# kvas7andy/unreal

Measured on AMD Instinct MI355X. Metric: env-steps/sec (whole node), UNREAL maze 84x84, higher is better.
Workload: dtype f32 (fp16x2-split MFMA operands, fp32 accumulate)

## Files before the change

include/unreal_hip.h:

```cpp
#ifndef UNREAL_HIP_H
#define UNREAL_HIP_H
#include <stdint.h>
#ifdef __cplusplus
extern "C" {
#endif

#define UNREAL_FRAME_BYTES 21168
#define UNREAL_PC_CELLS 400
#define UNREAL_GEMM_RELU 1
#define UNREAL_GEMM_ACCUM 2
#define UNREAL_GEMM_ATOMIC 4
#define UNREAL_GEMM_RELU_MASK 8
#define UNREAL_GEMM_RELU_BITS 16

int unreal_maze_step(int B, int H1, const int* actions, const int* active, int* pos, int* last_action,
                     float* last_reward, int* count, uint8_t* frames, float* r_reward, int* r_action,
                     int* r_terminal, int* r_last_action, float* r_last_reward, float* r_pc,
                     float* out_reward, int* out_terminal, float* episode_reward, float* score_out,
                     int* score_valid, int reset_on_terminal, int track_score, void* stream);
int unreal_maze_rollout_step(int B, int H1, const int* actions, int* pos, int* last_action, float* last_reward, int* count,
                             uint8_t* frames, float* r_reward, int* r_action, int* r_terminal, int* r_last_action,
                             float* r_last_reward, float* r_pc, float* out_reward, int* out_terminal,
                             float* episode_reward, float* score_out, int* score_valid, int* active,
                             int* active_log_t, int* n_steps, int* terminal_end, int* next_idx ,
// ... 88 lines not shown
int unreal_encoder_hw_fwd(int N, int H, int W, const uint8_t* frames, long frame_stride, const int* frame_idx,
                          float frame_scale, const float* W1, const float* b1, const float* W2, const float* b2,
                          float* c1_out, float* f2_out, float* f2_absmax, void* stream);
int unreal_encoder_hw_bwd(int N, int H, int W, const uint8_t* frames, long frame_stride, const int* frame_idx,
                          float frame_scale, const float* W2, const float* c1_saved, const float* d2, float* work,
                          long work_floats, float* dW1, float* db1, float* dW2, float* db2, void* stream);
int unreal_encoder_hw_work_floats(int N, int H, int W, long* out, void* stream);

int unreal_gemm_f32(int transA, int transB, int M, int N, int K, const float* A, int lda, const float* B,
                    int ldb, float* C, int ldc, const float* bias, const float* mask, int ldm, int flags,
                    int splitk, void* stream);
int unreal_absmax_f32(int rows, int cols, const float* x, int ld, float* slot, void* stream);
int unreal_gemm_f32_split_nt(int M, int N, int K, const float* A, int lda, const float* a_absmax, const uint16_t* W2,
                             int ldw, long plane_stride, const float* w_absmax, float* C, int ldc, float* c_absmax,
                             const float* bias,
                             const void* mask ,
                             int ldm, int flags, int splitk, void* stream);
int unreal_gemm_f32_split_nt_slabs(int M, int N, int K, const float* A, int lda, const float* a_absmax, const uint16_t* W3,
                                   int ldw, long plane_stride, const float* w_absmax, float* C, int ldc, float* c_absmax,
                                   const float* bias, int flags, int splitk, float* partials, long partial_floats,
                                   void* stream);
int unreal_gemm_f32_split_tn(int M, int N, int K, const float* A, int lda, const float* a_absmax, const float* B, int ldb,
                             const float* b_absmax, float* C, int ldc, float* colsum, int splitk, void* stream);
int unreal_shadow_refresh_multi(const void* abs_descs, int n_abs, int abs_blocks, const void* split_descs, int n_split,
                                int split_blocks, void* stream);
int unreal_split_f16x2(int rows, int cols, const float* src, int ld_src, int transpose, int row_perm, uint16_t* dst,
                       int ld_dst, long plane_stride, const float* w_absmax, void* stream);
int unreal_lstm_step_fwd(int rows, const float* x, int ldx, int Kx, const float* x_absmax, const float* h_prev, int ld_hprev,
                         const uint16_t* W2, int ldw, long plane_stride, const float* w_absmax, float* gates,
                         const float* bias, const float* c_prev, float* c_out, float* h_out, int ld_h, void* stream);
int unreal_lstm_bptt_step(int rows, const float* d_gates, const float* a_absmax, const uint16_t* Wh2, int ldw,
                          long plane_stride, const float* w_absmax, const float* dh_above, float* dc_io,
                          const float* gates_act, const float* c_prev, const float* c_new, float* dpre,
                          float* dpre_absmax0, float* dpre_absmax1, void* stream);
int unreal_lstm_gates_fwd(int rows, const float* pre, const float* bias, const float* c_prev, float* gates_act,
                          float* c_out, float* h_out, int ld_h, void* stream);
int unreal_lstm_gates_bwd(int rows, const float* dh_above, const float* dh_rec, float* dc_io, const float* gates_act,
                          const float* c_prev, const float* c_new, float* dpre, float* dpre_absmax0 ,
                          float* dpre_absmax1 , void* stream);

int unreal_linear_small_fwd(int rows, int K, int NOUT, const float* X, int ldx, const float* W, const float* b,
                            float* out, int ldo, void* stream);
int unreal_linear_small_bwd(int rows, int K, int NOUT, const float* X, int ldx, const float* dO, int ldo,
                            const float* W, float* dX, int lddx, int accumulate_dx, float* dW, int dw_stride_k,
                            int dw_stride_n, float* db, void* stream);
int unreal_softmax_sample(int rows, int A, float* logits_pi, int ld, const double* u, int* action, void* stream);
// ... 38 lines not shown
```

unreal_amd/csrc/gemm_split.hip:

```cpp
#include "common.h"

namespace {

constexpr int BK = 32;
constexpr int NPL = 2;
typedef _Float16 f16x8 __attribute__((ext_vector_type(8)));
typedef _Float16 f16x2 __attribute__((ext_vector_type(2)));
constexpr int ROW_B = 80;
constexpr int FLAG_RELU = 1, FLAG_ACCUM = 2, FLAG_ATOMIC = 4, FLAG_RELU_MASK = 8, FLAG_RELU_BITS = 16;

typedef float f32x2 __attribute__((ext_vector_type(2)));
typedef unsigned int u32x2 __attribute__((ext_vector_type(2)));
typedef unsigned int u32x4 __attribute__((ext_vector_type(4)));

__device__ __forceinline__ int row_deal(int j) { return (j & ~7) | ((j & 1) << 2) | ((j >> 1) & 3); }

struct SplitArgs {
  int M, N, K;
  const float* A; int lda;
  const unsigned short* W; int ldw; long plane;
  float* C; int ldc;
  const float* bias;
  const float* mask; int ldm;
  int flags;
// ... 463 lines not shown
  }
  if (p.c_absmax0) {
    float* wmx0 = reinterpret_cast<float*>(smem_all + C_BYTES);
    omax = wave_max(omax);
    if ((threadIdx.x & 63) == 0) wmx0[threadIdx.x >> 6] = omax;
    __syncthreads();
    if (threadIdx.x < 64) {
      float m = wmx0[0];
#pragma unroll
      for (int g = 1; g < 4 * KW; ++g) m = fmaxf(m, wmx0[g]);
      absmax_commit(p.c_absmax0, m);
    }
  }
}

struct SplitTnArgs {
  int M, N, K;
  const float* A; int lda;
  const float* B; int ldb;
  float* C; int ldc;
  float* colsum;
  int ntx, nty, splitk, ktiles_per_split;
  const float* a_absmax; const float* b_absmax;
};

__device__ __forceinline__ int tn_m4() {
  const int t = threadIdx.x;
  return ((t >> 1) & 1) | (((t >> 4) & 1) << 1) | (((t >> 2) & 3) << 2) | (((t >> 5) & 1) << 4);
}
__device__ __forceinline__ int tn_k4() {
  const int t = threadIdx.x;
  return (t & 1) | ((t >> 6) << 1);
}

__device__ __forceinline__ void tn_piece_load(const float* __restrict__ P, int ld, int K, int c0, int k0, f32x4 (&reg)[4]) {
  const int m4 = tn_m4(), k4 = tn_k4();
  const int col = min(c0 + 4 * m4, ld - 4);
#pragma unroll
  for (int kk = 0; kk < 4; ++kk) {
    const int k = min(k0 + 4 * k4 + kk, K - 1);
    reg[kk] = *reinterpret_cast<const f32x4*>(P + (size_t)k * ld + col);
  }
}

template <int ROWS, bool RAGGED>
__device__ __forceinline__ void tn_piece_store(unsigned char* S, const f32x4 (&reg)[4], int klim, float scale) {
// ... 5 lines not shown
  for (int j = 0; j < 4; ++j) {
    const int r = 4 * m4 + j;
    u32x2 pl[NPL];
    split4_terms(ok[0] ? reg[0][j] * scale : 0.f, ok[1] ? reg[1][j] * scale : 0.f, ok[2] ? reg[2][j] * scale : 0.f,
                 ok[3] ? reg[3][j] * scale : 0.f, pl);
    const int off = (((k4 >> 1) ^ ((r >> 4) & 3)) * 2 + (k4 & 1)) * 8;
#pragma unroll
    for (int t = 0; t < NPL; ++t)
      *reinterpret_cast<u32x2*>(S + (t * ROWS + r) * ROW_B + off) = pl[t];
  }
}

template <bool RAGGED>
__device__ __forceinline__ void tn_colsum_acc(const f32x4 (&reg)[4], int klim, float w, float (&cs)[4]) {
  const int k4 = tn_k4();
#pragma unroll
  for (int kk = 0; kk < 4; ++kk) {
    const float wk = (!RAGGED || 4 * k4 + kk < klim) ? w : 0.f;
#pragma unroll
    for (int j = 0; j < 4; ++j) cs[j] = fmaf(wk, reg[kk][j], cs[j]);
  }
}

template <bool RAGGED>
__global__ __launch_bounds__(256, 2) void gemm_split_tn_kernel(SplitTnArgs p) {
  constexpr int BM = 128, BN = 128, TM = 2, TN = 2;
  constexpr int A_BYTES = NPL * BM * ROW_B, B_BYTES = NPL * BN * ROW_B;
  constexpr int OP_BYTES = A_BYTES + B_BYTES;
  __shared__ __attribute__((aligned(16))) unsigned char smem[OP_BYTES > 8 * BN * 4 ? OP_BYTES : 8 * BN * 4];
  const float SA = pow2_scale(*p.a_absmax), SB = pow2_scale(*p.b_absmax);
  const float INV_A = pow2_inv(SA), INV_B = pow2_inv(SB);
  unsigned char* As = smem;
  unsigned char* Bs = smem + A_BYTES;

  const int L = blockIdx.x, xcd = L & 7, s = L >> 3;
  const int tiles = p.ntx * p.nty;
  const int slab = (s / tiles) * 8 + xcd, tile = s % tiles;
  if (slab >= p.splitk) return;
  const int bx = tile % p.ntx, by = tile / p.ntx;
  const int m0 = by * BM, n0 = bx * BN;
  const int nk_total = (p.K + BK - 1) / BK;
  const int kt0 = slab * p.ktiles_per_split, kt1 = min(nk_total, kt0 + p.ktiles_per_split);
  if (kt0 >= kt1) return;
  const int nkt = kt1 - kt0;
  const int lane = threadIdx.x & 63, wave = threadIdx.x >> 6;
  const int wm = wave >> 1, wn = wave & 1;
  const int li = lane & 31, kh = lane >> 5;

  f32x16 acc[TM][TN];
#pragma unroll
  for (int i = 0; i < TM; ++i)
#pragma unroll
    for (int j = 0; j < TN; ++j)
#pragma unroll
      for (int r = 0; r < 16; ++r) acc[i][j][r] = 0.f;

  constexpr int TN_FLUSH = 8;
  f32x16 tot[TM][TN];
#pragma unroll
  for (int i = 0; i < TM; ++i)
#pragma unroll
    for (int j = 0; j < TN; ++j)
#pragma unroll
      for (int r = 0; r < 16; ++r) tot[i][j][r] = 0.f;
  f32x4 ra[4], rb[4];
  const float csw = (p.colsum != nullptr && by == 0) ? 1.f : 0.f;
  float cs[4] = {0.f, 0.f, 0.f, 0.f};
  tn_piece_load(p.A, p.lda, p.K, m0, kt0 * BK, ra);
  tn_piece_load(p.B, p.ldb, p.K, n0, kt0 * BK, rb);
  tn_piece_store<BM, RAGGED>(As, ra, p.K - kt0 * BK, SA);
  tn_piece_store<BN, RAGGED>(Bs, rb, p.K - kt0 * BK, SB);
  tn_colsum_acc<RAGGED>(rb, p.K - kt0 * BK, csw, cs);
  {
    const int k1 = (kt0 + min(1, nkt - 1)) * BK;
    tn_piece_load(p.A, p.lda, p.K, m0, k1, ra);
    tn_piece_load(p.B, p.ldb, p.K, n0, k1, rb);
  }
  __syncthreads();

  for (int it = 0; it < nkt; ++it) {
    f16x8 af[TM][NPL], bf[TN][NPL];
    read_frags<BM, BN, true>(As, Bs, wm, wn, li, kh, 0, af, bf);
    mma_frags<TM, TN>(af, bf, acc);
    read_frags<BM, BN, true>(As, Bs, wm, wn, li, kh, 1, af, bf);
    __syncthreads();
    const int kcur = (kt0 + min(it + 1, nkt - 1)) * BK, knext = (kt0 + min(it + 2, nkt - 1)) * BK;
    tn_piece_store<BM, RAGGED>(As, ra, p.K - kcur, SA);
    tn_piece_load(p.A, p.lda, p.K, m0, knext, ra);
    tn_piece_store<BN, RAGGED>(Bs, rb, p.K - kcur, SB);
    tn_colsum_acc<RAGGED>(rb, p.K - kcur, (it + 1 < nkt) ? csw : 0.f, cs);
    tn_piece_load(p.B, p.ldb, p.K, n0, knext, rb);
    mma_frags<TM, TN>(af, bf, acc);
    if ((it + 1) % TN_FLUSH == 0) {
#pragma unroll
      for (int i = 0; i < TM; ++i)
#pragma unroll
        for (int j = 0; j < TN; ++j)
#pragma unroll
          for (int r = 0; r < 16; ++r) { tot[i][j][r] += acc[i][j][r]; acc[i][j][r] = 0.f; }
    }
    __syncthreads();
  }
#pragma unroll
  for (int i = 0; i < TM; ++i)
#pragma unroll
    for (int j = 0; j < TN; ++j)
#pragma unroll
      for (int r = 0; r < 16; ++r) acc[i][j][r] += tot[i][j][r];

  if (csw != 0.f) {
    float* red = reinterpret_cast<float*>(smem);
    const int m4 = tn_m4(), k4 = tn_k4();
#pragma unroll
    for (int j = 0; j < 4; ++j) red[k4 * BN + 4 * m4 + j] = cs[j];
    __syncthreads();
    if (threadIdx.x < BN && n0 + threadIdx.x < p.N) {
      float v = 0.f;
#pragma unroll
      for (int k = 0; k < 8; ++k) v += red[k * BN + threadIdx.x];
      atomicAdd(p.colsum + n0 + threadIdx.x, v);
    }
  }
#pragma unroll
  for (int i = 0; i < TM; ++i)
#pragma unroll
// ... 9 lines not shown
}

__global__ __launch_bounds__(256) void split_planes_f16x2_kernel(int rows, int cols, const float* __restrict__ src, int ld_src,
                                                                 int transpose, unsigned short* __restrict__ dst, int ld_dst,
                                                                 long plane, int row_perm, const float* __restrict__ w_absmax) {
  __shared__ float t[32][33];
  const float sw = pow2_scale(*w_absmax);
  const int c0 = blockIdx.x * 32, r0 = blockIdx.y * 32;
  const int tx = threadIdx.x & 31, ty = threadIdx.x >> 5;
  for (int y = ty; y < 32; y += 8)
    if (r0 + y < rows && c0 + tx < cols) t[y][tx] = src[(size_t)(r0 + y) * ld_src + c0 + tx];
  __syncthreads();
  for (int y = ty; y < 32; y += 8) {
    int orow = transpose ? c0 + y : r0 + y;
    const int ocol = transpose ? r0 + tx : c0 + tx;
    if (row_perm == 1) orow = ((orow & 255) >> 4) * 64 + (orow >> 8) * 16 + (orow & 15);
    const bool ok = transpose ? (c0 + y < cols && r0 + tx < rows) : (r0 + y < rows && c0 + tx < cols);
    if (!ok) continue;
    const float x = (transpose ? t[tx][y] : t[y][tx]) * sw;
    const _Float16 h = (_Float16)x;
    const _Float16 l = (_Float16)(x - (float)h);
    dst[(size_t)orow * ld_dst + ocol] = __builtin_bit_cast(unsigned short, h);
    dst[plane + (size_t)orow * ld_dst + ocol] = __builtin_bit_cast(unsigned short, l);
  }
}

__global__ __launch_bounds__(256) void absmax_kernel(int rows, int cols, const float* __restrict__ x, int ld, float* slot) {
  float m = 0.f;
  if (ld == cols && (cols & 3) == 0 && ((((uintptr_t)x) & 15) == 0)) {
    const long n4 = (long)rows * cols / 4;
    const f32x4* x4 = reinterpret_cast<const f32x4*>(x);
    for (long i = (long)blockIdx.x * 256 + threadIdx.x; i < n4; i += (long)gridDim.x * 256) {
      const f32x4 v = x4[i];
      m = fmaxf(fmaxf(m, fmaxf(fabsf(v[0]), fabsf(v[1]))), fmaxf(fabsf(v[2]), fabsf(v[3])));
    }
  } else {
    const int wave = (blockIdx.x * 256 + threadIdx.x) >> 6, nw = (gridDim.x * 256) >> 6, lane = threadIdx.x & 63;
    for (int r = wave; r < rows; r += nw)
      for (int c = lane; c < cols; c += 64) m = fmaxf(m, fabsf(x[(size_t)r * ld + c]));
  }
  __shared__ float wm[4];
  m = wave_max(m);
  if ((threadIdx.x & 63) == 0) wm[threadIdx.x >> 6] = m;
  __syncthreads();
  if (threadIdx.x < 64) absmax_commit(slot, fmaxf(fmaxf(wm[0], wm[1]), fmaxf(wm[2], wm[3])));
}
// ... 292 lines not shown
  a.bias = nullptr; a.mask = nullptr; a.ldm = 0; a.flags = 0; a.vecA = 1;
  a.c_prev = c_prev; a.c_out = nullptr; a.h_out = nullptr; a.ld_h = 0;
  a.A2 = nullptr; a.lda2 = 0; a.K1 = 1024; a.K1pad = 0;
  a.dh_above = dh_above; a.dc_io = dc_io; a.gates_act = gates_act; a.c_new = c_new; a.dpre = dpre;
  a.a_absmax = a_absmax; a.a_floor = 0.f; a.w_absmax = w_absmax; a.c_absmax0 = dpre_absmax0; a.c_absmax1 = dpre_absmax1;
  a.splitk = 1; a.ktiles_per_split = 1024 / BK; a.slab_stride = 0;
  a.nbx = 4; a.nby = (rows + 63) / 64;
  const int grid = a.nbx * ((a.nby + 7) / 8 * 8);
  const long tiles = (long)a.nbx * a.nby;
  const int kw = tiles <= 256 ? 4 : tiles <= 512 ? 2 : 1;
  if (kw == 4) {
    UNREAL_LAUNCHED("bptt kw4");
    hipLaunchKernelGGL((gemm_split_nt_kernel<64, 64, true, 2, 4>), dim3(grid), dim3(1024), 0, (hipStream_t)stream, a);
  } else if (kw == 2) {
    UNREAL_LAUNCHED("bptt kw2");
    hipLaunchKernelGGL((gemm_split_nt_kernel<64, 64, true, 2, 2>), dim3(grid), dim3(512), 0, (hipStream_t)stream, a);
  } else {
    UNREAL_LAUNCHED("bptt kw1");
    hipLaunchKernelGGL((gemm_split_nt_kernel<64, 64, true, 2, 1>), dim3(grid), dim3(256), 0, (hipStream_t)stream, a);
  }
  return unreal_launch_status();
}

int unreal_gemm_f32_split_tn(int M, int N, int K, const float* A, int lda, const float* a_absmax, const float* B, int ldb,
                             const float* b_absmax, float* C, int ldc, float* colsum, int splitk, void* stream) {
  if (M <= 0 || N <= 0 || K <= 0 || !A || !B || !C || lda < M || ldb < N || ldc < N) return UNREAL_EINVAL;
  if ((lda & 3) || (ldb & 3) || lda < 4 || ldb < 4 || (((uintptr_t)A) & 15) || (((uintptr_t)B) & 15)) return UNREAL_EINVAL;
  SplitTnArgs a;
  a.M = M; a.N = N; a.K = K; a.A = A; a.lda = lda; a.B = B; a.ldb = ldb; a.C = C; a.ldc = ldc; a.colsum = colsum;
  a.a_absmax = a_absmax; a.b_absmax = b_absmax;
  if (!a.a_absmax || !a.b_absmax) return UNREAL_EINVAL;
  a.ntx = (N + 127) / 128; a.nty = (M + 127) / 128;
  const int nk = (K + BK - 1) / BK;
  if (splitk < 1) splitk = 1;
  if (splitk > nk) splitk = nk;
  a.ktiles_per_split = (nk + splitk - 1) / splitk;
  a.splitk = (nk + a.ktiles_per_split - 1) / a.ktiles_per_split;
  const long grid = (long)a.ntx * a.nty * ((a.splitk + 7) / 8 * 8);
  if (grid > 0x7fffffffL) return UNREAL_EINVAL;
  if (K % BK == 0) {
    UNREAL_LAUNCHED("split_tn even");
    hipLaunchKernelGGL(gemm_split_tn_kernel<false>, dim3((unsigned)grid), dim3(256), 0, (hipStream_t)stream, a);
  } else {
    UNREAL_LAUNCHED("split_tn ragged");
    hipLaunchKernelGGL(gemm_split_tn_kernel<true>, dim3((unsigned)grid), dim3(256), 0, (hipStream_t)stream, a);
  }
  return unreal_launch_status();
}

}
```

unreal_amd/model/model.py:

```python
import math
from collections import OrderedDict

import numpy as np
import torch

from .. import ops

ALIGN = 64
XLD = 264


def xcat_ld(action_size, objective_size=0):
    return max(XLD, (256 + action_size + 1 + objective_size + 7) // 8 * 8)


def _small_chunks(n):
    out = []
    while n > 0:
        w = n if n in (1, 3, 4, 5, 6, 7) else (1 if n == 2 else (7 if n >= 10 else n - 3 if n - 3 in (3, 4, 5, 6) else 4))
        out.append(w)
        n -= w
    return out


# ... 59 lines not shown
        self.frame_idx = torch.zeros(rows, dtype=torch.int32, device=device)
        self.c1 = f(rows * c1_dim) if save_c1 else None
        self.f2 = f(rows * f2_dim)
        self.f2_bits = torch.zeros(rows * ops.RELU_WORDS, dtype=torch.int16, device=device) \
            if save_c1 and f2_dim == ops.F2_DIM and c1_dim == ops.C1_DIM else None
        self.xcat = torch.zeros(rows * xld, dtype=torch.float32, device=device)
        if lstm:
            self.gates = f(rows * 1024)
            self.c = f(rows * 256)
            self.h = f(rows * 256)
            self.c0 = torch.zeros(B * 256, dtype=torch.float32, device=device)
            self.h0 = torch.zeros(B * 256, dtype=torch.float32, device=device)


class GradWS(object):

    def __init__(self, rows, B, device, lstm=True, pc=True, A=4, pc_rows=None, f2_dim=ops.F2_DIM):
        f = lambda n: torch.empty(n, dtype=torch.float32, device=device)
        pc_rows = rows if pc_rows is None else pc_rows
        self.f2_dim = f2_dim
        self.d_feat = f(rows * 256)
        self.d_fc = f(rows * 256)
        self.d_f2 = f(rows * f2_dim)
        if lstm:
            self.d_gates = f(rows * 1024)
            self.dh_rec = f(B * 256)
            self.dc = f(B * 256)
        self.rows, self.lstm, self.device = rows, lstm, device
        self.hp = self.d_hp = self.d_dec = self.pc_R = None
        if pc:
            self.ensure_pc(pc_rows, A, own_d_hp=pc_rows != rows)

    def ensure_pc(self, pc_rows, A, own_d_hp=False):
        if self.hp is not None and self.hp.numel() >= pc_rows * ops.F2_DIM:
            return
        f = lambda n: torch.empty(n, dtype=torch.float32, device=self.device)
        self.hp = f(pc_rows * ops.F2_DIM)
        self.d_hp = f(pc_rows * ops.F2_DIM) if own_d_hp else None
        self.d_dec = None
        self.pc_R = f(pc_rows * ops.PC_CELLS)

    def ensure_d_dec(self, pc_rows, A):
        n = pc_rows * ops.PC_CELLS * (1 + A)
        if self.d_dec is None or self.d_dec.numel() < n:
            self.d_dec = torch.empty(n, dtype=torch.float32, device=self.device)
        return self.d_dec

    def ensure_rows(self, rows, B, device):
        if rows <= self.rows:
            return
        f = lambda n: torch.empty(n, dtype=torch.float32, device=device)
        self.rows = rows
        self.d_feat, self.d_fc, self.d_f2 = f(rows * 256), f(rows * 256), f(rows * self.f2_dim)
        if self.lstm:
            self.d_gates = f(rows * 1024)


def _splitk(M, N, K):
    tiles = ((M + 127) // 128) * ((N + 127) // 128)
    nk = (K + 31) // 32
    if nk < 64:
        return max(1, min(nk // 4 if nk >= 8 else 1, (1024 + tiles - 1) // tiles))
    return max(8, min(8 * int(round(128.0 / tiles)), nk // 4 // 8 * 8))


class UnrealModel(object):

    def __init__(self, action_size, objective_size, thread_index, use_lstm, use_pixel_change,
                 use_value_replay, use_reward_prediction, pixel_change_lambda, entropy_beta, device,
                 segnet_param_dict=None, image_shape=(84, 84), is_training=True, n_classes=0,
                 segnet_lambda=1.0, dropout=0.0, for_display=False, frame_scale=None, seed=0):
        if objective_size < 0:
            raise ValueError("objective_size must be >= 0")
        if segnet_param_dict is not None and segnet_param_dict.get("segnet_mode", 0) not in (0, None):
            raise NotImplementedError("only the vanilla encoder (segnet_mode == 0) is on the hot path")
        self.image_shape = (int(image_shape[0]), int(image_shape[1]))
# ... 329 lines not shown
                              splitk=_splitk(256, 1024, rows), colsum=g["lstm_bias"],
                              a_max=ws.s_x, b_max=s_all)
            c0 = 256
            for w in _small_chunks(K_x - 256):
                ops.linear_small_bwd(rows, 1024, w, gws.d_gates, 1024, ws.xcat[c0:], self.xld, None, None, 0, False,
                                     dW[c0 * 1024:], None, dw_stride_k=1, dw_stride_n=1024)
                c0 += w
            if T > 1:
                r1 = (T - 1) * B
                ops.gemm_split_tn(256, 1024, r1, ws.h, 256, gws.d_gates[B * 1024:], 1024, dW[K_x * 1024:], 1024,
                              splitk=_splitk(256, 1024, r1), a_max=self._one, b_max=s_all)
            if h0_nonzero:
                ops.gemm_split_tn(256, 1024, B, ws.h0, 256, gws.d_gates, 1024, dW[K_x * 1024:], 1024,
                              splitk=_splitk(256, 1024, B), a_max=self._one, b_max=s_all)
            s_dfc = self.new_slot()
            ops.gemm_split_nt(rows, 256, 1024, gws.d_gates, 1024, sh["lstm_fc_dgrad"], gws.d_fc, 256, mask=ws.xcat,
                              ldm=self.xld, flags=ops.GEMM_RELU_MASK, a_max=s_all, c_max=s_dfc)
            d_fc = gws.d_fc
        else:
            ops.relu_mask(rows, 256, d_feat, 256, ws.xcat, self.xld)
            d_fc = d_feat
            s_dfc = ops.absmax(rows, 256, d_fc, 256, self.new_slot())
        F = self.F
        ops.gemm_split_tn(F, 256, rows, ws.f2, F, d_fc, 256, g["W_base_fc1"], 256,
                              splitk=_splitk(F, 256, rows), colsum=g["b_base_fc1"], a_max=ws.s_f2, b_max=s_dfc)
        s_df2 = self.new_slot()
        if ws.f2_bits is not None and self.relu_bits:
            ops.gemm_split_nt(rows, F, 256, d_fc, 256, sh["fc1_dgrad"], gws.d_f2, F, mask=ws.f2_bits,
                              ldm=ops.RELU_WORDS, flags=ops.GEMM_RELU_BITS, a_max=s_dfc, c_max=s_df2)
        else:
            ops.gemm_split_nt(rows, F, 256, d_fc, 256, sh["fc1_dgrad"], gws.d_f2, F, mask=ws.f2, ldm=F,
                              flags=ops.GEMM_RELU_MASK, a_max=s_dfc, c_max=s_df2)
        self.encoder_backward(ring, ws.frame_idx[:rows], ws.c1, gws.d_f2, c1_max=ws.s_c1, d2_max=s_df2)

    def heads_forward(self, rows, feat, ld, pi_out, v_out):
        p, A = self.p, self._action_size
        ops.linear_small_fwd(rows, 256, A, feat, ld, p["W_base_fc_p"], p["b_base_fc_p"], pi_out, A)
        ops.linear_small_fwd(rows, 256, 1, feat, ld, p["W_base_fc_v"], p["b_base_fc_v"], v_out, 1)

    def policy_step(self, rows, feat, ld, u, pi_out, v_out, actions_out):
        p = self.p
        ops.policy_step(rows, self._action_size, feat, ld, p["W_base_fc_p"], p["b_base_fc_p"], p["W_base_fc_v"],
                        p["b_base_fc_v"], u, pi_out, v_out, actions_out)

    def value_forward(self, rows, feat, ld, v_out):
        p = self.p
        ops.linear_small_fwd(rows, 256, 1, feat, ld, p["W_base_fc_v"], p["b_base_fc_v"], v_out, 1)

# ... 104 lines not shown
```

unreal_amd/ops.py:

```python
import torch

from ._lib import lib, ptr, stream

FRAME_BYTES = 21168
PC_CELLS = 400
F2_DIM = 2592
C1_DIM = 6400
GEMM_RELU, GEMM_ACCUM, GEMM_ATOMIC, GEMM_RELU_MASK, GEMM_RELU_BITS = 1, 2, 4, 8, 16
RELU_WORDS = 162

FRAME_SHAPE = (84, 84)
FRAME_HW_MIN, FRAME_HW_MAX = 20, 480


def frame_dims(H, W):
    H, W = int(H), int(W)
    if not (FRAME_HW_MIN <= H <= FRAME_HW_MAX and FRAME_HW_MIN <= W <= FRAME_HW_MAX):
        raise ValueError("frame size %dx%d: supported are %d <= H, W <= %d" % (H, W, FRAME_HW_MIN, FRAME_HW_MAX))
    h1, w1 = (H - 8) // 4 + 1, (W - 8) // 4 + 1
    h2, w2 = (h1 - 4) // 2 + 1, (w1 - 4) // 2 + 1
    return h1, w1, h2, w2, 32 * h2 * w2


def frame_stride(H, W):
# ... 615 lines not shown


def gemm_split_nt_slabs(M, N, K, A, lda, W, C, ldc, partials, splitk, bias=None, flags=0, a_max=None, c_max=None):
    if W.N != N or W.K != K:
        raise ValueError("split weights are [%d,%d], GEMM wants [%d,%d]" % (W.N, W.K, N, K))
    _chk(A, "f32", (M - 1) * lda + K, "A"); _chk(C, "f32", (M - 1) * ldc + N, "C")
    _chk(bias, "f32", N, "bias", optional=True); _chk(partials, "f32", splitk * M * ((N + 3) // 4 * 4), "partials")
    _chk(a_max, "f32", 1, "a_max", optional=True); _chk(c_max, "f32", 1, "c_max", optional=True)
    a_max = _absmax_of(A, M, K, lda, a_max)
    _call("unreal_gemm_f32_split_nt_slabs", M, N, K, ptr(A), lda, ptr(a_max), ptr(W.planes), W.ldw, W.plane, ptr(W.wmax), ptr(C),
          ldc, ptr(c_max), ptr(bias), flags, splitk, ptr(partials), partials.numel())


def gemm_split_tn(M, N, K, A, lda, B, ldb, C, ldc, splitk=1, colsum=None, a_max=None, b_max=None):
    _chk(A, "f32", (K - 1) * lda + M, "A"); _chk(B, "f32", (K - 1) * ldb + N, "B"); _chk(C, "f32", (M - 1) * ldc + N, "C")
    _chk(colsum, "f32", N, "colsum", optional=True)
    _chk(a_max, "f32", 1, "a_max", optional=True); _chk(b_max, "f32", 1, "b_max", optional=True)
    a_max = _absmax_of(A, K, M, lda, a_max)
    b_max = _absmax_of(B, K, N, ldb, b_max)
    _call("unreal_gemm_f32_split_tn", M, N, K, ptr(A), lda, ptr(a_max), ptr(B), ldb, ptr(b_max), ptr(C), ldc, ptr(colsum),
          splitk)


def lstm_step_fwd(rows, h_prev, Wh, gates, bias, c_prev, c_out, h_out, ld_hprev=256, ld_h=256, x=None, ldx=0, Kx=0,
                  x_max=None):
    kxpad = (Kx + 31) // 32 * 32 if x is not None else 0
    if Wh.N != 1024 or Wh.K != kxpad + 256 or Wh.row_perm != 1:
        raise ValueError("lstm_step_fwd needs the gate-interleaved [1024,%d] shadow of the LSTM kernel" % (kxpad + 256))
    _chk(h_prev, "f32", (rows - 1) * ld_hprev + 256, "h_prev"); _chk(gates, "f32", rows * 1024, "gates")
    _chk(bias, "f32", 1024, "bias"); _chk(c_prev, "f32", rows * 256, "c_prev"); _chk(c_out, "f32", rows * 256, "c_out")
    _chk(h_out, "f32", (rows - 1) * ld_h + 256, "h_out")
    _chk(x, "f32", (rows - 1) * ldx + Kx if x is not None else None, "x", optional=True)
    _chk(x_max, "f32", 1, "x_max", optional=True)
    if x is not None:
        x_max = _absmax_of(x, rows, Kx, ldx, x_max)
    _call("unreal_lstm_step_fwd", rows, ptr(x), ldx, Kx, ptr(x_max), ptr(h_prev), ld_hprev, ptr(Wh.planes), Wh.ldw, Wh.plane,
          ptr(Wh.wmax), ptr(gates), ptr(bias), ptr(c_prev), ptr(c_out), ptr(h_out), ld_h)


def lstm_gates_fwd(rows, pre, bias, c_prev, gates_act, c_out, h_out, ld_h=256):
    _chk(pre, "f32", rows * 1024); _chk(bias, "f32", 1024); _chk(c_prev, "f32", rows * 256)
    _chk(gates_act, "f32", rows * 1024, optional=True); _chk(c_out, "f32", rows * 256)
    _chk(h_out, "f32", (rows - 1) * ld_h + 256)
    _call("unreal_lstm_gates_fwd", rows, ptr(pre), ptr(bias), ptr(c_prev), ptr(gates_act), ptr(c_out), ptr(h_out),
          ld_h)

# ... 149 lines not shown
```

unreal_amd/train/trainer.py:

```python
import time

import torch

from .. import ops
from ..environment.environment import Environment
from ..environment.maze_environment import BatchedMazeEnvironment
from ..model.model import UnrealModel, PathWS, GradWS
from .experience import Experience

PERFORMANCE_LOG_INTERVAL = 2000


def log_uniform(lo, hi, rate):
    import math
    return math.exp(math.log(lo) * (1 - rate) + math.log(hi) * rate)


class PhiloxDraws(object):

    def __init__(self, seed, rank=0, batch=None, world_size=1):
        self.seed = int(seed)
        self.counter = 1
        self.batch = None if batch is None else int(batch)
        self.stride = None if batch is None else int(batch) * int(world_size)
# ... 469 lines not shown
                          g["W_pc_deconv_v"], g["b_pc_deconv_v"], g["W_pc_deconv_a"], g["b_pc_deconv_a"], dhp_max=s_dhp,
                          hp_max=s_hp, ddec_max=s_dd)
        return s_dhp

    def _train_pc(self):
        B, Ta, A, net = self.Bg, self.local_t_max, self.action_size, self.local_network
        p, g, gws = net.p, net.g, self.gws
        rows = Ta * B
        ws = self.aux_ws
        gws.ensure_pc(rows, A)
        feat, ld = self._sample_sequence()
        s_bhp = net.new_slot()
        net.pc_head_forward(B, feat, ld, self.boot_hp, ws=self.boot_ws, hp_max=s_bhp)
        ops.pc_deconv_fwd(B, A, self.boot_hp, p["W_pc_deconv_v"], p["b_pc_deconv_v"], p["W_pc_deconv_a"],
                          p["b_pc_deconv_a"], qmax=self.boot_qmax, hp_max=s_bhp)
        ops.pc_returns(self.ring, Ta + 1, self.seq_idx, self.seq_len, self.boot_qmax, self.gamma_pc, gws.pc_R)
        feat, ld = self._aux_forward()
        s_hp = net.new_slot()
        net.pc_head_forward(rows, feat, ld, gws.hp, ws=self.aux_ws, hp_max=s_hp)
        ops.gather_i32(self.ring.r_action, self.aux_ws.frame_idx[:rows], self.seq_act)
        d_hp = gws.d_f2
        s_dhp = self._pc_deconv_loss_backward(gws, rows, self.seq_mask, d_hp, s_hp)
        from ..model.model import _splitk
        ops.gemm_split_tn(256, 2592, rows, feat, ld, d_hp, 2592, g["W_pc_fc1"], 2592,
                              splitk=_splitk(256, 2592, rows), colsum=g["b_pc_fc1"],
                              a_max=net._one if self.use_lstm else self.aux_ws.s_x, b_max=s_dhp)
        ops.gemm_split_nt(rows, 256, 2592, d_hp, 2592, net.shadow["pc_fc1_dgrad"], gws.d_feat, 256, a_max=s_dhp)
        net.trunk_backward(self.ring, self.aux_ws, gws, Ta, B, gws.d_feat)

    def _train_vr(self):
        B, Ta, net = self.Bg, self.local_t_max, self.local_network
        p, g, gws = net.p, net.g, self.gws
        rows = Ta * B
        ws = self.aux_ws
        feat, ld = self._sample_sequence()
        net.value_forward(B, feat, ld, self.aux_boot_v)
        ops.vr_returns(self.ring, Ta + 1, self.seq_idx, self.seq_len, self.aux_boot_v, self.gamma, self.aux_R)
        feat, ld = self._aux_forward()
        net.value_forward(rows, feat, ld, self.aux_v)
        ops.vr_loss_grad(rows, self.aux_v, self.aux_R, self.seq_mask, self.grad_scale, self.dv, self.losses[4:5])
        ops.linear_small_bwd(rows, 256, 1, feat, ld, self.dv, 1, p["W_base_fc_v"], gws.d_feat, 256, False,
                             g["W_base_fc_v"], g["b_base_fc_v"])
        net.trunk_backward(self.ring, self.aux_ws, gws, Ta, B, gws.d_feat)

    batch_aux_default = True

    def _train_aux_batched(self):
        B, Ta, A, net = self.Bg, self.local_t_max, self.action_size, self.local_network
        p, g, gws, sh = net.p, net.g, self.gws2, net.shadow
# ... 3 lines not shown
            ops.replay_sample_seq(self.ring, L, self.seq_start2[s], self.seq_idx2[s], self.seq_len2[s])
            ops.seq_last_idx(B, self.seq_idx2[s], self.seq_len2[s], self.last2[s * B:(s + 1) * B])
            ops.seq_mask(B, Ta, self.seq_len2[s], self.seq_mask2[s])
        bw = self.boot2_ws
        ops.gather_i32(self.last2, self.map_boot, bw.frame_idx[:2 * B])
        feat, ld = net.trunk_forward(self.ring, bw, 1, 2 * B, lar_from_ring=True, save_c1=False)
        s_bhp = net.new_slot()
        net.pc_head_forward(B, feat, 2 * ld, self.boot_hp, ws=self.boot2_ws, hp_max=s_bhp)
        ops.pc_deconv_fwd(B, A, self.boot_hp, p["W_pc_deconv_v"], p["b_pc_deconv_v"], p["W_pc_deconv_a"],
                          p["b_pc_deconv_a"], qmax=self.boot_qmax, hp_max=s_bhp)
        ops.pc_returns(self.ring, L, self.seq_idx2[0], self.seq_len2[0], self.boot_qmax, self.gamma_pc, gws.pc_R)
        net.value_forward(B, feat[ld:], 2 * ld, self.aux_boot_v)
        ops.vr_returns(self.ring, L, self.seq_idx2[1], self.seq_len2[1], self.aux_boot_v, self.gamma, self.aux_R)
        ws = self.aux2_ws
        ops.gather_i32(self.seq_idx_cat, self.map_seq, ws.frame_idx[:2 * rows])
        feat, ld = net.trunk_forward(self.ring, ws, Ta, 2 * B, lar_from_ring=True, save_c1=True)
        d_feat = gws.d_feat
        s_hp = net.new_slot()
        net.pc_head_forward(rows, feat, 2 * ld, gws.hp, ws=self.aux2_ws, hp_max=s_hp)
        ops.gather_i32(self.ring.r_action, self.seq_idx2[0][:rows], self.seq_act)
        d_hp = gws.d_hp
        s_dhp = self._pc_deconv_loss_backward(gws, rows, self.seq_mask2[0], d_hp, s_hp)
        from ..model.model import _splitk
        ops.gemm_split_tn(256, 2592, rows, feat, 2 * ld, d_hp, 2592, g["W_pc_fc1"], 2592,
                          splitk=_splitk(256, 2592, rows), colsum=g["b_pc_fc1"],
                          a_max=net._one if self.use_lstm else self.aux2_ws.s_x, b_max=s_dhp)
        ops.gemm_split_nt(rows, 256, 2592, d_hp, 2592, sh["pc_fc1_dgrad"], d_feat, 2 * 256, a_max=s_dhp)
        net.value_forward(rows, feat[ld:], 2 * ld, self.aux_v)
        ops.vr_loss_grad(rows, self.aux_v, self.aux_R, self.seq_mask2[1], self.grad_scale, self.aux_dv, self.losses[4:5])
        ops.linear_small_bwd(rows, 256, 1, feat[ld:], 2 * ld, self.aux_dv, 1, p["W_base_fc_v"], d_feat[256:], 2 * 256, False,
                             g["W_base_fc_v"], g["b_base_fc_v"])
        net.trunk_backward(self.ring, ws, gws, Ta, 2 * B, d_feat)

    def _train_rp(self):
        B, net, ws = self.Bg, self.local_network, self.rp_ws
        p, g, gws = net.p, net.g, self.gws
        self.draws.randint(2, self.rp_coin)
        self.draws.uniform(self.rp_u)
        ops.replay_sample_rp(self.ring, self.rp_coin, self.rp_u, ws.frame_idx[:3 * B], self.rp_class, self.rp_mode)
        s_c1 = net.new_slot()
        F = net.F
        net.encoder_forward(self.ring, ws.frame_idx[:3 * B], ws.f2, ws.c1, c1_max=s_c1, ws=ws)
        ops.linear_small_fwd(B, 3 * F, 3, ws.f2, 3 * F, p["W_rp_fc1"], p["b_rp_fc1"], self.rp_logits, 3)
        ops.rp_loss_grad(B, self.rp_logits, self.rp_class, self.grad_scale, None, self.rp_dlogits,
                         self.losses[5:6])
        ops.linear_small_bwd(B, 3 * F, 3, ws.f2, 3 * F, self.rp_dlogits, 3, p["W_rp_fc1"], gws.d_f2, 3 * F, False,
                             g["W_rp_fc1"], g["b_rp_fc1"])
        ops.relu_mask(3 * B, F, gws.d_f2, F, ws.f2, F)
        net.encoder_backward(self.ring, ws.frame_idx[:3 * B], ws.c1, gws.d_f2,
# ... 92 lines not shown
```

Baseline: 3.762 million.

## Pre-split narrow activation operand into fp16x2 planes for weight-gradient TN GEMMs

Adds a kernel that transposes a narrow (256-wide) fp32 activation or gradient matrix once into K-contiguous fp16 hi/lo planes, optionally folding in the bias column sum. The TN weight-gradient GEMM gains template variants that load the pre-split planes directly into shared memory instead of re-splitting fp32 tiles in every block. This targets the redundant split and transposed fp32 loads repeated across the wide grid dimension. The cost is an extra launch and a plane buffer write and read.

```diff
diff --git a/include/unreal_hip.h b/include/unreal_hip.h
--- a/include/unreal_hip.h
+++ b/include/unreal_hip.h
@@ -134,6 +134,11 @@
                                    void* stream);
 int unreal_gemm_f32_split_tn(int M, int N, int K, const float* A, int lda, const float* a_absmax, const float* B, int ldb,
                              const float* b_absmax, float* C, int ldc, float* colsum, int splitk, void* stream);
+int unreal_split_act_f16x2(int K, int N, const float* src, int ld_src, const float* absmax, uint16_t* dst, int ld_dst,
+                           long plane_stride, float* colsum, void* stream);
+int unreal_gemm_f32_split_tn_planes(int M, int N, int K, const float* A, int lda, const uint16_t* Ap, int ldap, long a_plane,
+                                    const float* a_absmax, const float* B, int ldb, const uint16_t* Bp, int ldbp, long b_plane,
+                                    const float* b_absmax, float* C, int ldc, float* colsum, int splitk, void* stream);
 int unreal_shadow_refresh_multi(const void* abs_descs, int n_abs, int abs_blocks, const void* split_descs, int n_split,
                                 int split_blocks, void* stream);
 int unreal_split_f16x2(int rows, int cols, const float* src, int ld_src, int transpose, int row_perm, uint16_t* dst,
diff --git a/unreal_amd/csrc/gemm_split.hip b/unreal_amd/csrc/gemm_split.hip
--- a/unreal_amd/csrc/gemm_split.hip
+++ b/unreal_amd/csrc/gemm_split.hip
@@ -509,6 +509,8 @@
   float* colsum;
   int ntx, nty, splitk, ktiles_per_split;
   const float* a_absmax; const float* b_absmax;
+  const unsigned short* Ap; int ldap; long a_plane;
+  const unsigned short* Bp; int ldbp; long b_plane;
 };
 
 __device__ __forceinline__ int tn_m4() {
@@ -560,7 +562,22 @@
   }
 }
 
-template <bool RAGGED>
+__device__ __forceinline__ void tn_planes_load(const unsigned short* __restrict__ P, int ld, long plane, int rows_total, int r0,
+                                               int k0, u32x4 (&reg)[4]) {
+#pragma unroll
+  for (int q = 0; q < 4; ++q) reg[q] = w_piece_load<128>(P, ld, plane, rows_total, r0, k0, q, threadIdx.x);
+}
+
+__device__ __forceinline__ void tn_planes_store(unsigned char* S, const u32x4 (&reg)[4]) {
+#pragma unroll
+  for (int q = 0; q < 4; ++q) {
+    const int id = threadIdx.x + 256 * q;
+    const int t = id / (128 * 4), r = row_deal((id / 4) % 128), c = id % 4;
+    *reinterpret_cast<u32x4*>(S + (t * 128 + r) * ROW_B + (c ^ ((r >> 4) & 3)) * 16) = reg[q];
+  }
+}
+
+template <bool RAGGED, bool PRE_A, bool PRE_B>
 __global__ __launch_bounds__(256, 2) void gemm_split_tn_kernel(SplitTnArgs p) {
   constexpr int BM = 128, BN = 128, TM = 2, TN = 2;
   constexpr int A_BYTES = NPL * BM * ROW_B, B_BYTES = NPL * BN * ROW_B;
@@ -602,17 +619,24 @@
 #pragma unroll
       for (int r = 0; r < 16; ++r) tot[i][j][r] = 0.f;
   f32x4 ra[4], rb[4];
-  const float csw = (p.colsum != nullptr && by == 0) ? 1.f : 0.f;
+  u32x4 pa[4], pb[4];
+  const float csw = (!PRE_B && p.colsum != nullptr && by == 0) ? 1.f : 0.f;
   float cs[4] = {0.f, 0.f, 0.f, 0.f};
-  tn_piece_load(p.A, p.lda, p.K, m0, kt0 * BK, ra);
-  tn_piece_load(p.B, p.ldb, p.K, n0, kt0 * BK, rb);
-  tn_piece_store<BM, RAGGED>(As, ra, p.K - kt0 * BK, SA);
-  tn_piece_store<BN, RAGGED>(Bs, rb, p.K - kt0 * BK, SB);
-  tn_colsum_acc<RAGGED>(rb, p.K - kt0 * BK, csw, cs);
+#define TN_LOAD_A(k) { if constexpr (PRE_A) tn_planes_load(p.Ap, p.ldap, p.a_plane, p.M, m0, k, pa); \
+                       else tn_piece_load(p.A, p.lda, p.K, m0, k, ra); }
+#define TN_LOAD_B(k) { if constexpr (PRE_B) tn_planes_load(p.Bp, p.ldbp, p.b_plane, p.N, n0, k, pb); \
+                       else tn_piece_load(p.B, p.ldb, p.K, n0, k, rb); }
+#define TN_STORE_A(k) { if constexpr (PRE_A) tn_planes_store(As, pa); else tn_piece_store<BM, RAGGED>(As, ra, p.K - (k), SA); }
+#define TN_STORE_B(k) { if constexpr (PRE_B) tn_planes_store(Bs, pb); else tn_piece_store<BN, RAGGED>(Bs, rb, p.K - (k), SB); }
+  TN_LOAD_A(kt0 * BK)
+  TN_LOAD_B(kt0 * BK)
+  TN_STORE_A(kt0 * BK)
+  TN_STORE_B(kt0 * BK)
+  if constexpr (!PRE_B) tn_colsum_acc<RAGGED>(rb, p.K - kt0 * BK, csw, cs);
   {
     const int k1 = (kt0 + min(1, nkt - 1)) * BK;
-    tn_piece_load(p.A, p.lda, p.K, m0, k1, ra);
-    tn_piece_load(p.B, p.ldb, p.K, n0, k1, rb);
+    TN_LOAD_A(k1)
+    TN_LOAD_B(k1)
   }
   __syncthreads();
 
@@ -623,11 +647,12 @@
     read_frags<BM, BN, true>(As, Bs, wm, wn, li, kh, 1, af, bf);
     __syncthreads();
     const int kcur = (kt0 + min(it + 1, nkt - 1)) * BK, knext = (kt0 + min(it + 2, nkt - 1)) * BK;
-    tn_piece_store<BM, RAGGED>(As, ra, p.K - kcur, SA);
-    tn_piece_load(p.A, p.lda, p.K, m0, knext, ra);
-    tn_piece_store<BN, RAGGED>(Bs, rb, p.K - kcur, SB);
-    tn_colsum_acc<RAGGED>(rb, p.K - kcur, (it + 1 < nkt) ? csw : 0.f, cs);
-    tn_piece_load(p.B, p.ldb, p.K, n0, knext, rb);
+    TN_STORE_A(kcur)
+    TN_LOAD_A(knext)
+    TN_STORE_B(kcur)
+    if constexpr (!PRE_B)
+      tn_colsum_acc<RAGGED>(rb, p.K - kcur, (it + 1 < nkt) ? csw : 0.f, cs);
+    TN_LOAD_B(knext)
     mma_frags<TM, TN>(af, bf, acc);
     if ((it + 1) % TN_FLUSH == 0) {
 #pragma unroll
@@ -639,6 +664,10 @@
     }
     __syncthreads();
   }
+#undef TN_STORE_B
+#undef TN_STORE_A
+#undef TN_LOAD_B
+#undef TN_LOAD_A
 #pragma unroll
   for (int i = 0; i < TM; ++i)
 #pragma unroll
@@ -694,6 +723,67 @@
     const _Float16 l = (_Float16)(x - (float)h);
     dst[(size_t)orow * ld_dst + ocol] = __builtin_bit_cast(unsigned short, h);
     dst[plane + (size_t)orow * ld_dst + ocol] = __builtin_bit_cast(unsigned short, l);
+  }
+}
+
+constexpr int ACT_KT = 128, ACT_KCH = 512;
+
+__global__ __launch_bounds__(256) void split_act_planes_kernel(int K, int N, const float* __restrict__ src, int ld_src, int vec,
+                                                               const float* __restrict__ absmax, unsigned short* __restrict__ dst,
+                                                               int ld_dst, long plane, float* __restrict__ colsum) {
+  __shared__ float t[ACT_KT][33];
+  const float scale = pow2_scale(*absmax);
+  const int n0 = blockIdx.x * 32, kb = blockIdx.y * ACT_KCH;
+  const int kend = min(kb + ACT_KCH, (K + BK - 1) / BK * BK);
+  const int lr = threadIdx.x >> 3, lc = (threadIdx.x & 7) * 4;
+  const int sn = threadIdx.x >> 3, sk = (threadIdx.x & 7) * 16;
+  float cs[4] = {0.f, 0.f, 0.f, 0.f};
+  for (int k0 = kb; k0 < kend; k0 += ACT_KT) {
+    f32x4 v[ACT_KT / 32];
+#pragma unroll
+    for (int j = 0; j < ACT_KT / 32; ++j) {
+      const int k = k0 + lr + 32 * j, col = n0 + lc;
+      const float* row = src + (size_t)k * ld_src + col;
+      if (k < K && vec && col + 3 < N) {
+        v[j] = *reinterpret_cast<const f32x4*>(row);
+      } else {
+#pragma unroll
+        for (int e = 0; e < 4; ++e) v[j][e] = (k < K && col + e < N) ? row[e] : 0.f;
+      }
+    }
+#pragma unroll
+    for (int j = 0; j < ACT_KT / 32; ++j)
+#pragma unroll
+      for (int e = 0; e < 4; ++e) {
+        cs[e] += v[j][e];
+        t[lr + 32 * j][lc + e] = v[j][e];
+      }
+    __syncthreads();
+    if (n0 + sn < N && k0 + sk < kend) {
+      u32x2 pl[4][NPL];
+#pragma unroll
+      for (int q = 0; q < 4; ++q)
+        split4_terms(t[sk + 4 * q][sn] * scale, t[sk + 4 * q + 1][sn] * scale, t[sk + 4 * q + 2][sn] * scale,
+                     t[sk + 4 * q + 3][sn] * scale, pl[q]);
+      unsigned short* d = dst + (size_t)(n0 + sn) * ld_dst + k0 + sk;
+#pragma unroll
+      for (int pt = 0; pt < NPL; ++pt) {
+        u32x4* o = reinterpret_cast<u32x4*>(d + pt * plane);
+        o[0] = (u32x4){pl[0][pt][0], pl[0][pt][1], pl[1][pt][0], pl[1][pt][1]};
+        o[1] = (u32x4){pl[2][pt][0], pl[2][pt][1], pl[3][pt][0], pl[3][pt][1]};
+      }
+    }
+    __syncthreads();
+  }
+  if (colsum) {
+#pragma unroll
+    for (int e = 0; e < 4; ++e) t[lr][lc + e] = cs[e];
+    __syncthreads();
+    if (threadIdx.x < 32 && n0 + (int)threadIdx.x < N) {
+      float s = 0.f;
+      for (int r = 0; r < 32; ++r) s += t[r][threadIdx.x];
+      atomicAdd(colsum + n0 + threadIdx.x, s);
+    }
   }
 }
 
@@ -1032,30 +1122,80 @@
   return unreal_launch_status();
 }
 
+static int split_tn_grid(SplitTnArgs& a, int splitk, unsigned* grid) {
+  a.ntx = (a.N + 127) / 128; a.nty = (a.M + 127) / 128;
+  const int nk = (a.K + BK - 1) / BK;
+  if (splitk < 1) splitk = 1;
+  if (splitk > nk) splitk = nk;
+  a.ktiles_per_split = (nk + splitk - 1) / splitk;
+  a.splitk = (nk + a.ktiles_per_split - 1) / a.ktiles_per_split;
+  const long g = (long)a.ntx * a.nty * ((a.splitk + 7) / 8 * 8);
+  if (g > 0x7fffffffL) return UNREAL_EINVAL;
+  *grid = (unsigned)g;
+  return UNREAL_OK;
+}
+
 int unreal_gemm_f32_split_tn(int M, int N, int K, const float* A, int lda, const float* a_absmax, const float* B, int ldb,
                              const float* b_absmax, float* C, int ldc, float* colsum, int splitk, void* stream) {
   if (M <= 0 || N <= 0 || K <= 0 || !A || !B || !C || lda < M || ldb < N || ldc < N) return UNREAL_EINVAL;
   if ((lda & 3) || (ldb & 3) || lda < 4 || ldb < 4 || (((uintptr_t)A) & 15) || (((uintptr_t)B) & 15)) return UNREAL_EINVAL;
-  SplitTnArgs a;
+  SplitTnArgs a = {};
   a.M = M; a.N = N; a.K = K; a.A = A; a.lda = lda; a.B = B; a.ldb = ldb; a.C = C; a.ldc = ldc; a.colsum = colsum;
   a.a_absmax = a_absmax; a.b_absmax = b_absmax;
   if (!a.a_absmax || !a.b_absmax) return UNREAL_EINVAL;
-  a.ntx = (N + 127) / 128; a.nty = (M + 127) / 128;
-  const int nk = (K + BK - 1) / BK;
-  if (splitk < 1) splitk = 1;
-  if (splitk > nk) splitk = nk;
-  a.ktiles_per_split = (nk + splitk - 1) / splitk;
-  a.splitk = (nk + a.ktiles_per_split - 1) / a.ktiles_per_split;
-  const long grid = (long)a.ntx * a.nty * ((a.splitk + 7) / 8 * 8);
-  if (grid > 0x7fffffffL) return UNREAL_EINVAL;
+  unsigned grid;
+  if (split_tn_grid(a, splitk, &grid) != UNREAL_OK) return UNREAL_EINVAL;
   if (K % BK == 0) {
     UNREAL_LAUNCHED("split_tn even");
-    hipLaunchKernelGGL(gemm_split_tn_kernel<false>, dim3((unsigned)grid), dim3(256), 0, (hipStream_t)stream, a);
+    hipLaunchKernelGGL((gemm_split_tn_kernel<false, false, false>), dim3(grid), dim3(256), 0, (hipStream_t)stream, a);
   } else {
     UNREAL_LAUNCHED("split_tn ragged");
-    hipLaunchKernelGGL(gemm_split_tn_kernel<true>, dim3((unsigned)grid), dim3(256), 0, (hipStream_t)stream, a);
+    hipLaunchKernelGGL((gemm_split_tn_kernel<true, false, false>), dim3(grid), dim3(256), 0, (hipStream_t)stream, a);
   }
   return unreal_launch_status();
 }
 
-}
+int unreal_split_act_f16x2(int K, int N, const float* src, int ld_src, const float* absmax, uint16_t* dst, int ld_dst,
+                           long plane_stride, float* colsum, void* stream) {
+  if (K <= 0 || N <= 0 || !src || !absmax || !dst || ld_src < N) return UNREAL_EINVAL;
+  const int kpad = (K + BK - 1) / BK * BK;
+  if (ld_dst < kpad || (ld_dst & 7) || (plane_stride & 7) || plane_stride < (long)N * ld_dst || (((uintptr_t)dst) & 15))
+    return UNREAL_EINVAL;
+  const int vec = (ld_src & 3) == 0 && (((uintptr_t)src) & 15) == 0;
+  dim3 grid((N + 31) / 32, (kpad + ACT_KCH - 1) / ACT_KCH);
+  hipLaunchKernelGGL(split_act_planes_kernel, grid, dim3(256), 0, (hipStream_t)stream, K, N, src, ld_src, vec, absmax, dst,
+                     ld_dst, plane_stride, colsum);
+  return unreal_launch_status();
+}
+
+static bool planes_ok(const uint16_t* P, int ld, long plane, int rows, int K) {
+  return !((((uintptr_t)P) & 15) || (ld & 7) || ld < (K + BK - 1) / BK * BK || (plane & 7) || plane < (long)rows * ld);
+}
+
+int unreal_gemm_f32_split_tn_planes(int M, int N, int K, const float* A, int lda, const uint16_t* Ap, int ldap, long a_plane,
+                                    const float* a_absmax, const float* B, int ldb, const uint16_t* Bp, int ldbp, long b_plane,
+                                    const float* b_absmax, float* C, int ldc, float* colsum, int splitk, void* stream) {
+  if (M <= 0 || N <= 0 || K <= 0 || !C || ldc < N || !a_absmax || !b_absmax) return UNREAL_EINVAL;
+  if (!A == !Ap || !B == !Bp || (!Ap && !Bp)) return UNREAL_EINVAL;
+  if (A && (lda < M || (lda & 3) || lda < 4 || (((uintptr_t)A) & 15))) return UNREAL_EINVAL;
+  if (B && (ldb < N || (ldb & 3) || ldb < 4 || (((uintptr_t)B) & 15))) return UNREAL_EINVAL;
+  if (Ap && !planes_ok(Ap, ldap, a_plane, M, K)) return UNREAL_EINVAL;
+  if (Bp && !planes_ok(Bp, ldbp, b_plane, N, K)) return UNREAL_EINVAL;
+  if (Bp && colsum) return UNREAL_EINVAL;
+  SplitTnArgs a = {};
+  a.M = M; a.N = N; a.K = K; a.A = A; a.lda = lda; a.B = B; a.ldb = ldb; a.C = C; a.ldc = ldc; a.colsum = colsum;
+  a.a_absmax = a_absmax; a.b_absmax = b_absmax;
+  a.Ap = Ap; a.ldap = ldap; a.a_plane = a_plane; a.Bp = Bp; a.ldbp = ldbp; a.b_plane = b_plane;
+  unsigned grid;
+  if (split_tn_grid(a, splitk, &grid) != UNREAL_OK) return UNREAL_EINVAL;
+  const bool ragged = K % BK != 0;
+#define LAUNCH_TN(R_, PA_, PB_) hipLaunchKernelGGL((gemm_split_tn_kernel<R_, PA_, PB_>), dim3(grid), dim3(256), 0, \
+                                                   (hipStream_t)stream, a)
+  if (Ap && Bp) LAUNCH_TN(false, true, true);
+  else if (Ap) { if (ragged) LAUNCH_TN(true, true, false); else LAUNCH_TN(false, true, false); }
+  else { if (ragged) LAUNCH_TN(true, false, true); else LAUNCH_TN(false, false, true); }
+#undef LAUNCH_TN
+  return unreal_launch_status();
+}
+
+}
diff --git a/unreal_amd/model/model.py b/unreal_amd/model/model.py
--- a/unreal_amd/model/model.py
+++ b/unreal_amd/model/model.py
@@ -105,6 +105,7 @@
         self.d_feat = f(rows * 256)
         self.d_fc = f(rows * 256)
         self.d_f2 = f(rows * f2_dim)
+        self.act_planes = torch.empty(ops.act_planes_numel(rows, 256), dtype=torch.int16, device=device)
         if lstm:
             self.d_gates = f(rows * 1024)
             self.dh_rec = f(B * 256)
@@ -135,6 +136,7 @@
         f = lambda n: torch.empty(n, dtype=torch.float32, device=device)
         self.rows = rows
         self.d_feat, self.d_fc, self.d_f2 = f(rows * 256), f(rows * 256), f(rows * self.f2_dim)
+        self.act_planes = torch.empty(ops.act_planes_numel(rows, 256), dtype=torch.int16, device=device)
         if self.lstm:
             self.d_gates = f(rows * 1024)
 
@@ -510,8 +512,9 @@
             d_fc = d_feat
             s_dfc = ops.absmax(rows, 256, d_fc, 256, self.new_slot())
         F = self.F
-        ops.gemm_split_tn(F, 256, rows, ws.f2, F, d_fc, 256, g["W_base_fc1"], 256,
-                              splitk=_splitk(F, 256, rows), colsum=g["b_base_fc1"], a_max=ws.s_f2, b_max=s_dfc)
+        dfc_planes = ops.split_act_f16x2(rows, 256, d_fc, 256, gws.act_planes, s_dfc, colsum=g["b_base_fc1"])
+        ops.gemm_split_tn_planes(F, 256, rows, ws.f2, F, dfc_planes, 0, g["W_base_fc1"], 256,
+                                 splitk=_splitk(F, 256, rows), a_max=ws.s_f2)
         s_df2 = self.new_slot()
         if ws.f2_bits is not None and self.relu_bits:
             ops.gemm_split_nt(rows, F, 256, d_fc, 256, sh["fc1_dgrad"], gws.d_f2, F, mask=ws.f2_bits,
diff --git a/unreal_amd/ops.py b/unreal_amd/ops.py
--- a/unreal_amd/ops.py
+++ b/unreal_amd/ops.py
@@ -661,6 +661,51 @@
           splitk)
 
 
+class ActPlanes(object):
+
+    def __init__(self, buf, K, N, wmax):
+        self.K, self.N, self.wmax = K, N, wmax
+        self.ld = (K + 31) // 32 * 32
+        self.plane = N * self.ld
+        _chk(buf, "i16", 2 * self.plane, "planes")
+        self.planes = buf
+
+
+def act_planes_numel(K, N):
+    return 2 * N * ((K + 31) // 32 * 32)
+
+
+def split_act_f16x2(K, N, src, ld_src, buf, wmax, colsum=None):
+    _chk(src, "f32", (K - 1) * ld_src + N, "src"); _chk(wmax, "f32", 1, "wmax", optional=True)
+    _chk(colsum, "f32", N, "colsum", optional=True)
+    wmax = _absmax_of(src, K, N, ld_src, wmax)
+    P = ActPlanes(buf, K, N, wmax)
+    _call("unreal_split_act_f16x2", K, N, ptr(src), ld_src, ptr(wmax), ptr(P.planes), P.ld, P.plane, ptr(colsum))
+    return P
+
+
+def gemm_split_tn_planes(M, N, K, A, lda, B, ldb, C, ldc, splitk=1, colsum=None, a_max=None, b_max=None):
+    pa, pb = isinstance(A, ActPlanes), isinstance(B, ActPlanes)
+    if not (pa or pb):
+        raise ValueError("gemm_split_tn_planes: neither operand is pre-split (use gemm_split_tn)")
+    for P, rows, name in ((A, M, "A"), (B, N, "B")):
+        if isinstance(P, ActPlanes) and (P.K != K or P.N != rows):
+            raise ValueError("%s planes are [%d][%d], the product wants [%d][%d]" % (name, P.K, P.N, K, rows))
+    if not pa:
+        _chk(A, "f32", (K - 1) * lda + M, "A"); _chk(a_max, "f32", 1, "a_max", optional=True)
+        a_max = _absmax_of(A, K, M, lda, a_max)
+    if not pb:
+        _chk(B, "f32", (K - 1) * ldb + N, "B"); _chk(b_max, "f32", 1, "b_max", optional=True)
+        b_max = _absmax_of(B, K, N, ldb, b_max)
+    _chk(C, "f32", (M - 1) * ldc + N, "C"); _chk(colsum, "f32", N, "colsum", optional=True)
+    _call("unreal_gemm_f32_split_tn_planes", M, N, K,
+          None if pa else ptr(A), 0 if pa else lda, ptr(A.planes) if pa else None, A.ld if pa else 0, A.plane if pa else 0,
+          ptr(A.wmax) if pa else ptr(a_max),
+          None if pb else ptr(B), 0 if pb else ldb, ptr(B.planes) if pb else None, B.ld if pb else 0, B.plane if pb else 0,
+          ptr(B.wmax) if pb else ptr(b_max),
+          ptr(C), ldc, ptr(colsum), splitk)
+
+
 def lstm_step_fwd(rows, h_prev, Wh, gates, bias, c_prev, c_out, h_out, ld_hprev=256, ld_h=256, x=None, ldx=0, Kx=0,
                   x_max=None):
     kxpad = (Kx + 31) // 32 * 32 if x is not None else 0
diff --git a/unreal_amd/train/trainer.py b/unreal_amd/train/trainer.py
--- a/unreal_amd/train/trainer.py
+++ b/unreal_amd/train/trainer.py
@@ -515,9 +515,10 @@
         d_hp = gws.d_f2
         s_dhp = self._pc_deconv_loss_backward(gws, rows, self.seq_mask, d_hp, s_hp)
         from ..model.model import _splitk
-        ops.gemm_split_tn(256, 2592, rows, feat, ld, d_hp, 2592, g["W_pc_fc1"], 2592,
-                              splitk=_splitk(256, 2592, rows), colsum=g["b_pc_fc1"],
-                              a_max=net._one if self.use_lstm else self.aux_ws.s_x, b_max=s_dhp)
+        feat_planes = ops.split_act_f16x2(rows, 256, feat, ld, gws.act_planes,
+                                          net._one if self.use_lstm else self.aux_ws.s_x)
+        ops.gemm_split_tn_planes(256, 2592, rows, feat_planes, 0, d_hp, 2592, g["W_pc_fc1"], 2592,
+                                 splitk=_splitk(256, 2592, rows), colsum=g["b_pc_fc1"], b_max=s_dhp)
         ops.gemm_split_nt(rows, 256, 2592, d_hp, 2592, net.shadow["pc_fc1_dgrad"], gws.d_feat, 256, a_max=s_dhp)
         net.trunk_backward(self.ring, self.aux_ws, gws, Ta, B, gws.d_feat)
 
@@ -567,9 +568,10 @@
         d_hp = gws.d_hp
         s_dhp = self._pc_deconv_loss_backward(gws, rows, self.seq_mask2[0], d_hp, s_hp)
         from ..model.model import _splitk
-        ops.gemm_split_tn(256, 2592, rows, feat, 2 * ld, d_hp, 2592, g["W_pc_fc1"], 2592,
-                          splitk=_splitk(256, 2592, rows), colsum=g["b_pc_fc1"],
-                          a_max=net._one if self.use_lstm else self.aux2_ws.s_x, b_max=s_dhp)
+        feat_planes = ops.split_act_f16x2(rows, 256, feat, 2 * ld, gws.act_planes,
+                                          net._one if self.use_lstm else self.aux2_ws.s_x)
+        ops.gemm_split_tn_planes(256, 2592, rows, feat_planes, 0, d_hp, 2592, g["W_pc_fc1"], 2592,
+                                 splitk=_splitk(256, 2592, rows), colsum=g["b_pc_fc1"], b_max=s_dhp)
         ops.gemm_split_nt(rows, 256, 2592, d_hp, 2592, sh["pc_fc1_dgrad"], d_feat, 2 * 256, a_max=s_dhp)
         net.value_forward(rows, feat[ld:], 2 * ld, self.aux_v)
         ops.vr_loss_grad(rows, self.aux_v, self.aux_R, self.seq_mask2[1], self.grad_scale, self.aux_dv, self.losses[4:5])
```

Result: no change. 3.760 million (median of 6 runs) (-0.1%).
